# ishine/dmel_codec

Measured on AMD Instinct MI355X. Metric: audio-sec/sec (encode+decode RTF) @24 kHz batch 32, higher is better.
Workload: dtype f32; 1 GPU; cfg2: encode+decode, 24000 Hz, 80 mel, 8 FSQ groups [7, 5, 5], WaveNet 20+20 layers, BigVGAN-base, batch 32 x 1 s per GPU; lanes=3, vocoder_streams=1

## Files before the change

dmel_codec_amd/_lib.py:

```python
from __future__ import annotations

import ctypes as C
import os
from typing import Optional, Sequence

import torch

_HERE = os.path.dirname(os.path.abspath(__file__))
LIB_PATH = os.environ.get("DMEL_LIB") or os.path.join(_HERE, "libdmel_hip.so")
_lib: Optional[C.CDLL] = None

i64p = C.POINTER(C.c_int64)
i32p = C.POINTER(C.c_int32)
f32p = C.POINTER(C.c_float)
vp = C.c_void_p
GRAD_READY_FN = C.CFUNCTYPE(None, vp, C.c_int64, C.c_int64)


class BigVGANConfig(C.Structure):
    _fields_ = [
        ("num_mels", C.c_int),
        ("upsample_initial_channel", C.c_int),
        ("num_upsamples", C.c_int),
        ("upsample_rates", C.c_int * 8),
# ... 10 lines not shown


PROTOTYPES = {
    "dmel_last_error": (C.c_char_p, []),
    "dmel_abi_version": (C.c_int, []),
    "dmel_stft_plan_create": (C.c_int, [C.POINTER(vp), C.c_int, C.c_int, C.c_int, C.c_int, C.c_int, C.c_double, C.c_double, vp]),
    "dmel_stft_plan_destroy": (None, [vp]),
    "dmel_mel_basis_host": (C.c_int, [C.c_int, C.c_int, C.c_int, C.c_double, C.c_double, vp]),
    "dmel_stft_plan_mel_basis": (C.c_int, [vp, vp]),
    "dmel_stft_num_frames": (C.c_int64, [vp, C.c_int64]),
    "dmel_stft_logmel_f32": (C.c_int, [vp, vp, C.c_int64, vp, vp, C.c_int, C.c_int64, vp]),
    "dmel_resample_f32": (C.c_int, [vp, vp, vp, C.c_int, C.c_int64, C.c_int64, C.c_int, C.c_int, C.c_int, vp]),
    "dmel_resample_window_f32": (C.c_int, [vp, C.c_int64, C.c_int64, C.c_int64, vp, vp, C.c_int, C.c_int64, C.c_int64, C.c_int64, C.c_int, C.c_int,
                                           C.c_int, vp]),
    "dmel_resample_window_items_f32": (C.c_int, [vp, C.c_int64, C.c_int64, i64p, i64p, vp, C.c_int64, i64p, vp, C.c_int64, i64p, C.c_int, i64p,
                                                 C.c_int, i64p, i64p, i64p, vp, vp]),
    "dmel_pcm_convert_items": (C.c_int, [C.POINTER(vp), i32p, C.POINTER(vp), i32p, i64p, C.c_int, vp, vp]),
    "dmel_pcm_convert_items_ch": (C.c_int, [C.POINTER(vp), i32p, i32p, i32p, C.POINTER(vp), i32p, i32p, i64p, C.c_int, vp, vp]),
    "dmel_stft_f32": (C.c_int, [vp, vp, C.c_int64, vp, vp, vp, C.c_int, C.c_int64, vp]),
    "dmel_stft_window_f32": (C.c_int, [vp, vp, C.c_int64, C.c_int64, C.c_int64, vp, vp, vp, C.c_int, C.c_int64, C.c_int64, C.c_int64, vp]),
    "dmel_stft_window_items_f32": (C.c_int, [vp, vp, C.c_int64, C.c_int64, i64p, i64p, vp, vp, vp, C.c_int, i64p, i64p, i64p, vp, vp]),
    "dmel_aa_snake_f32": (C.c_int, [vp, vp, vp, vp, vp, vp, C.c_int, C.c_int, C.c_int, C.c_int64, vp]),
    "dmel_aa_snake_items_f32": (C.c_int, [vp, vp, vp, vp, vp, vp, C.c_int, C.c_int, C.c_int, C.c_int64, vp, vp]),
    "dmel_aa_snake_backward_f32": (C.c_int, [vp, vp, vp, vp, vp, vp, vp, vp, vp, C.c_int, C.c_int, C.c_int, C.c_int64, vp]),
    "dmel_discriminator_create": (C.c_int, [C.POINTER(vp)]),
    "dmel_discriminator_destroy": (None, [vp]),
    "dmel_discriminator_set_tensor": (C.c_int, [vp, C.c_char_p, vp, C.POINTER(C.c_int64), C.c_int]),
    "dmel_discriminator_finalize": (C.c_int, [vp]),
    "dmel_discriminator_out_frames": (C.c_int64, [vp, C.c_int64]),
    "dmel_discriminator_workspace_bytes": (C.c_size_t, [vp, C.c_int, C.c_int, C.c_int64]),
    "dmel_discriminator_forward": (C.c_int, [vp, vp, vp, C.c_int, C.c_int, C.c_int64, vp, C.c_size_t, vp]),
    "dmel_discriminator_enable_training": (C.c_int, [vp, C.c_int]),
    "dmel_discriminator_set_train_precision": (C.c_int, [vp, C.c_int]),
    "dmel_discriminator_refresh": (C.c_int, [vp, C.c_int, C.POINTER(C.c_char_p), C.POINTER(vp), vp]),
    "dmel_discriminator_train_workspace_bytes": (C.c_size_t, [vp, C.c_int, C.c_int, C.c_int64]),
    "dmel_discriminator_grad_floats": (C.c_int64, [vp]),
    "dmel_discriminator_grad_slot": (C.c_int, [vp, C.c_char_p, C.POINTER(C.c_int64), C.POINTER(C.c_int64)]),
    "dmel_discriminator_forward_train": (C.c_int, [vp, vp, vp, C.c_int, C.c_int, C.c_int64, vp, C.c_size_t, vp]),
    "dmel_discriminator_backward": (C.c_int, [vp, vp, vp, vp, C.c_int, C.c_int, C.c_int64, vp, C.c_size_t, vp]),
    "dmel_convnext_create": (C.c_int, [C.POINTER(vp), C.c_int]),
    "dmel_convnext_destroy": (None, [vp]),
    "dmel_convnext_set_tensor": (C.c_int, [vp, C.c_char_p, vp, C.POINTER(C.c_int64), C.c_int]),
    "dmel_convnext_enable_training": (C.c_int, [vp, C.c_int]),
    "dmel_convnext_set_train_precision": (C.c_int, [vp, C.c_int]),
    "dmel_convnext_finalize": (C.c_int, [vp]),
    "dmel_convnext_workspace_bytes": (C.c_size_t, [vp, C.c_int, C.c_int64]),
# ... 171 lines not shown
```

dmel_codec_amd/csrc/aa_snake.hip:

```cpp
#include "ops.h"
#include "snake_dev.h"

namespace dmel {

constexpr int kSnakeTile = 1024;
constexpr int kSnakeFwdTile = 1008;

typedef float f32x4 __attribute__((ext_vector_type(4)));

template <bool VEC>
__device__ __forceinline__ void aa_snake_row(const float* __restrict__ xr, float* __restrict__ yr, const float* __restrict__ alpha,
                                             const float* __restrict__ beta, const Taps12& tu, const Taps12& td, int logscale, int c, int T,
                                             int first, int nsub, float* xs, float* ve, float* vo) {
  float a = alpha[c], bt = beta ? beta[c] : a;
  if (logscale) {
    bt = beta ? expf(bt) : expf(a);
    a = expf(a);
  }
  const float inv_b = 1.0f / (bt + 1e-9f);
  const int tid = threadIdx.x;
  auto fetch = [&](int t0) {
    const int s = t0 - 8 + 4 * tid;
    if (VEC && s >= 0 && s + 4 <= T) return *reinterpret_cast<const f32x4*>(xr + s);
    f32x4 v;
    v.x = xr[min(max(s, 0), T - 1)];
    v.y = xr[min(max(s + 1, 0), T - 1)];
    v.z = xr[min(max(s + 2, 0), T - 1)];
    v.w = xr[min(max(s + 3, 0), T - 1)];
    return v;
  };
  float aa[8], bb[8];
#pragma unroll
  for (int i = 0; i < 8; ++i) { aa[i] = a; bb[i] = inv_b; }
  f32x4 pre = {0.f, 0.f, 0.f, 0.f};
  if (first < T) pre = fetch(first);
  for (int sub = 0; sub < nsub; ++sub) {
    const int t0 = first + sub * kSnakeFwdTile;
    if (t0 >= T) break;
    const int len = min(kSnakeFwdTile, T - t0);
    if (sub) __syncthreads();
    *reinterpret_cast<f32x4*>(xs + 4 * tid) = pre;
    if (sub + 1 < nsub && t0 + kSnakeFwdTile < T) pre = fetch(t0 + kSnakeFwdTile);
    __syncthreads();
    if (4 * tid < len + 6) {
      float w[12];
      lds_read3_b128(xs + 4 * tid, w);
      float u[8];
#pragma unroll
      for (int i = 0; i < 4; ++i) {
        float ue = 0.f, uo = 0.f;
#pragma unroll
        for (int j = 0; j < 6; ++j) {
          ue = fmaf(tu.f[2 * j + 1], w[i + 7 - j], ue);
          uo = fmaf(tu.f[2 * j], w[i + 8 - j], uo);
        }
        u[2 * i] = ue;
        u[2 * i + 1] = uo;
      }
      snake_n(u, aa, bb);
      *reinterpret_cast<f32x4*>(ve + 4 * tid) = f32x4{u[0], u[2], u[4], u[6]};
      *reinterpret_cast<f32x4*>(vo + 4 * tid) = f32x4{u[1], u[3], u[5], u[7]};
    }
    __syncthreads();
    const int pe = T - t0 + 3;
    if (t0 == 0 || pe < len + 6) {
      if (tid < 3) {
        if (t0 == 0) ve[tid] = vo[tid] = ve[3];
        if (pe + tid < len + 6) ve[pe + tid] = vo[pe + tid] = vo[pe - 1];
      }
      __syncthreads();
    }
    if (4 * tid < len) {
      float e[12], o[12];
      lds_read3_b128(ve + 4 * tid, e);
      lds_read3_b128(vo + 4 * tid, o);
      f32x4 out;
#pragma unroll
      for (int i = 0; i < 4; ++i) {
        float acc = td.f[0] * o[i];
#pragma unroll
        for (int k = 1; k < 6; ++k) {
          acc = fmaf(td.f[2 * k - 1], e[i + k], acc);
          acc = fmaf(td.f[2 * k], o[i + k], acc);
        }
        out[i] = fmaf(td.f[11], e[i + 6], acc);
      }
      float* yp = yr + t0 + 4 * tid;
      if (VEC) {
        *reinterpret_cast<f32x4*>(yp) = out;
      } else {
#pragma unroll
        for (int i = 0; i < 4; ++i)
          if (4 * tid + i < len) yp[i] = out[i];
      }
    }
  }
}

template <bool VEC>
__global__ __launch_bounds__(256) void aa_snake_kernel(const float* __restrict__ x, float* __restrict__ y,
                                                          const float* __restrict__ alpha, const float* __restrict__ beta,
                                                          Taps12 tu, Taps12 td, int logscale, int C, int T, int nsub) {
  __shared__ __attribute__((aligned(16))) float xs[kSnakeFwdTile + 16];
  __shared__ __attribute__((aligned(16))) float ve[kSnakeFwdTile + 16];
  __shared__ __attribute__((aligned(16))) float vo[kSnakeFwdTile + 16];
  const int c = blockIdx.y, b = blockIdx.z;
  const int64_t row = ((int64_t)b * C + c) * T;
  aa_snake_row<VEC>(x + row, y + row, alpha, beta, tu, td, logscale, c, T, blockIdx.x * nsub * kSnakeFwdTile, nsub, xs, ve, vo);
}

__global__ __launch_bounds__(256) void aa_snake_items_kernel(const float* __restrict__ x, float* __restrict__ y,
                                                                const float* __restrict__ alpha, const float* __restrict__ beta,
                                                                Taps12 tu, Taps12 td, int logscale, int C, int T,
                                                                const int64_t* __restrict__ len, int nsub) {
  __shared__ __attribute__((aligned(16))) float xs[kSnakeFwdTile + 16];
  __shared__ __attribute__((aligned(16))) float ve[kSnakeFwdTile + 16];
  __shared__ __attribute__((aligned(16))) float vo[kSnakeFwdTile + 16];
  const int c = blockIdx.y, b = blockIdx.z;
  const int n = (int)min(max(len[b], (int64_t)0), (int64_t)T);
  const int first = blockIdx.x * nsub * kSnakeFwdTile;
  if (first >= n) return;
  const int64_t row = ((int64_t)b * C + c) * T;
  const float* xr = x + row;
  float* yr = y + row;
  const bool vec = n % 4 == 0 && (reinterpret_cast<uintptr_t>(xr) | reinterpret_cast<uintptr_t>(yr)) % 16 == 0;
  if (vec) aa_snake_row<true>(xr, yr, alpha, beta, tu, td, logscale, c, n, first, nsub, xs, ve, vo);
  else aa_snake_row<false>(xr, yr, alpha, beta, tu, td, logscale, c, n, first, nsub, xs, ve, vo);
}

template <bool PARAMS>
__global__ __launch_bounds__(256) void aa_snake_bwd_kernel(const float* __restrict__ x, const float* __restrict__ dy,
                                                            float* dx, const float* __restrict__ alpha,
                                                            const float* __restrict__ beta, float* __restrict__ dalpha,
                                                            float* __restrict__ dbeta, const float* __restrict__ radd, const float* racc,
                                                            Taps12 tu, Taps12 td, int logscale, int C, int T) {
  __shared__ float xs[kSnakeTile + 12];
  __shared__ float dys[kSnakeTile + 12];
  __shared__ float dvs[2 * (kSnakeTile + 6)];
  __shared__ float dxs[kSnakeTile];
  __shared__ float red[2][4];
  const int c = blockIdx.y, b = blockIdx.z, tid = threadIdx.x;
  const int t0 = blockIdx.x * kSnakeTile;
  const int len = min(kSnakeTile, T - t0);
  const float* xr = x + ((int64_t)b * C + c) * T;
  const float* dyr = dy + ((int64_t)b * C + c) * T;
  float* dxr = dx + ((int64_t)b * C + c) * T;
  float a = alpha[c], bt = beta ? beta[c] : a;
  if (logscale) {
    bt = beta ? expf(bt) : expf(a);
    a = expf(a);
// ... 131 lines not shown
                       (const float*)nullptr, tu, td, logscale, C, (int)T);
  }
  DMEL_HIP(hipGetLastError());
  return DMEL_OK;
}

int launch_aa_snake_bwd_input(const float* x, const float* dy, float* dx, const float* radd, const float* racc, const float* alpha,
                              const float* beta, const float* up_taps_host, const float* down_taps_host, int logscale, int B, int C,
                              int64_t T, hipStream_t s) {
  DMEL_CHECK_ARG(x && dy && dx && alpha && up_taps_host && down_taps_host, "aa_snake_backward_input: NULL argument");
  DMEL_CHECK_ARG(B > 0 && C > 0 && T > 0 && B <= 65535 && C <= 65535 && T < ((int64_t)1 << 29), "aa_snake_backward_input: bad shape");
  Taps12 tu, td;
  for (int i = 0; i < 12; ++i) { tu.f[i] = 2.f * up_taps_host[i]; td.f[i] = down_taps_host[i]; }
  dim3 grid((unsigned)((T + kSnakeTile - 1) / kSnakeTile), (unsigned)C, (unsigned)B);
  {
    ProfScope ps("aa_snake_bwd", s, 0.0, (12.0 + (radd ? 4.0 : 0.0) + (racc ? 4.0 : 0.0)) * (double)B * C * (double)T);
    hipLaunchKernelGGL(aa_snake_bwd_kernel<false>, grid, dim3(256), 0, s, x, dy, dx, alpha, beta, (float*)nullptr, (float*)nullptr, radd,
                       racc, tu, td, logscale, C, (int)T);
  }
  DMEL_HIP(hipGetLastError());
  return DMEL_OK;
}

int launch_aa_snake(const float* x, float* y, const float* alpha, const float* beta, const float* up_taps_host,
                    const float* down_taps_host, int logscale, int B, int C, int64_t T, hipStream_t s) {
  DMEL_CHECK_ARG(x && y && alpha && up_taps_host && down_taps_host, "aa_snake: NULL argument");
  DMEL_CHECK_ARG(B > 0 && C > 0 && T > 0 && B <= 65535 && C <= 65535 && T < ((int64_t)1 << 30), "aa_snake: bad shape");
  Taps12 tu, td;
  for (int i = 0; i < 12; ++i) { tu.f[i] = 2.f * up_taps_host[i]; td.f[i] = down_taps_host[i]; }
  constexpr int nsub = 3;
  constexpr int span = kSnakeFwdTile * nsub;
  dim3 grid((unsigned)((T + span - 1) / span), (unsigned)C, (unsigned)B);
  const bool vec = T % 4 == 0 && (reinterpret_cast<uintptr_t>(x) | reinterpret_cast<uintptr_t>(y)) % 16 == 0;
  {
    ProfScope ps("aa_snake", s, 0.0, 8.0 * (double)B * C * (double)T);
    if (vec) hipLaunchKernelGGL(aa_snake_kernel<true>, grid, dim3(256), 0, s, x, y, alpha, beta, tu, td, logscale, C, (int)T, nsub);
    else hipLaunchKernelGGL(aa_snake_kernel<false>, grid, dim3(256), 0, s, x, y, alpha, beta, tu, td, logscale, C, (int)T, nsub);
  }
  DMEL_HIP(hipGetLastError());
  return DMEL_OK;
}

int launch_aa_snake_items(const float* x, float* y, const float* alpha, const float* beta, const float* up_taps_host,
                          const float* down_taps_host, int logscale, int B, int C, int64_t T, const int64_t* len, hipStream_t s) {
  DMEL_CHECK_ARG(x && y && alpha && up_taps_host && down_taps_host && len, "aa_snake_items: NULL argument");
  DMEL_CHECK_ARG(B > 0 && C > 0 && T > 0 && B <= 65535 && C <= 65535 && T < ((int64_t)1 << 30), "aa_snake_items: bad shape");
  Taps12 tu, td;
  for (int i = 0; i < 12; ++i) { tu.f[i] = 2.f * up_taps_host[i]; td.f[i] = down_taps_host[i]; }
  constexpr int nsub = 3;
  constexpr int span = kSnakeFwdTile * nsub;
  dim3 grid((unsigned)((T + span - 1) / span), (unsigned)C, (unsigned)B);
  {
    ProfScope ps("aa_snake", s, 0.0, 8.0 * (double)B * C * (double)T);
    hipLaunchKernelGGL(aa_snake_items_kernel, grid, dim3(256), 0, s, x, y, alpha, beta, tu, td, logscale, C, (int)T, len, nsub);
  }
  DMEL_HIP(hipGetLastError());
  return DMEL_OK;
}

}

extern "C" int dmel_aa_snake_items_f32(const float* x, float* y, const float* alpha, const float* beta, const float* up_filter12_host,
                                       const float* down_filter12_host, int logscale, int B, int C, int64_t T, const int64_t* lengths_dev,
                                       void* stream) {
  return dmel::launch_aa_snake_items(x, y, alpha, beta, up_filter12_host, down_filter12_host, logscale, B, C, T, lengths_dev,
                                     (hipStream_t)stream);
}

extern "C" int dmel_aa_snake_backward_f32(const float* x, const float* dy, float* dx, const float* alpha, const float* beta,
                                          float* dalpha, float* dbeta, const float* up_filter12_host, const float* down_filter12_host,
                                          int logscale, int B, int C, int64_t T, void* stream) {
  return dmel::launch_aa_snake_bwd(x, dy, dx, alpha, beta, dalpha, dbeta, up_filter12_host, down_filter12_host, logscale, B, C, T,
                                   (hipStream_t)stream);
}

extern "C" int dmel_aa_snake_backward_input_f32(const float* x, const float* dy, const float* add , float* dx, const float* alpha,
                                                const float* beta, const float* up_filter12_host, const float* down_filter12_host,
                                                int logscale, int B, int C, int64_t T, void* stream) {
  return dmel::launch_aa_snake_bwd_input(x, dy, dx, add, nullptr, alpha, beta, up_filter12_host, down_filter12_host, logscale, B, C, T,
                                         (hipStream_t)stream);
}

extern "C" int dmel_aa_snake_f32(const float* x, float* y, const float* alpha, const float* beta, const float* up_filter12_host,
                                 const float* down_filter12_host, int logscale, int B, int C, int64_t T, void* stream) {
  return dmel::launch_aa_snake(x, y, alpha, beta, up_filter12_host, down_filter12_host, logscale, B, C, T, (hipStream_t)stream);
}
```

dmel_codec_amd/csrc/modules.hip:

```cpp
#include <cmath>
#include <cstdlib>
#include <map>
#include <memory>

#include "ops.h"

using namespace dmel;

namespace {

struct HostTensor {
  std::vector<float> v;
  std::vector<int64_t> shape;
  int64_t numel() const { return (int64_t)v.size(); }
};

struct TensorStore {
  std::map<std::string, HostTensor> t;
  int set(const char* key, const float* data, const int64_t* shape, int ndim) {
    DMEL_CHECK_ARG(key && data && shape && ndim >= 0 && ndim <= 4, "set_tensor: bad argument");
    HostTensor h;
    int64_t n = 1;
    for (int i = 0; i < ndim; ++i) { h.shape.push_back(shape[i]); n *= shape[i]; }
    h.v.assign(data, data + n);
// ... 2511 lines not shown
  float* ua = bufs[4];

  {
    ConvRun r = run_1seg(mel, c.num_mels, T, x, c.upsample_initial_channel, T, B);
    r.seg[0].in_len = len_at(0);
    r.precision = prec;
    DMEL_TRY(launch_conv(m->conv_pre, r, st));
  }
  int64_t Tc = T;
  int ch = c.upsample_initial_channel;
  for (int i = 0; i < c.num_upsamples; ++i) {
    const UpStage& us = m->ups[i];
    const int64_t Tn = Tc * us.u;
    DMEL_TRY(launch_up_stage(us, x, xu, B, Tc, prec, st, len_at(i)));
    ch = us.Cout;
    Tc = Tn;
    const int64_t bs = (int64_t)ch * Tc;
    const bool multi = m->multi;
    const int64_t* len = len_at(i + 1);
    if (multi) {
      DMEL_HIP(hipEventRecord(m->ev_fork, st));
      for (int k = 0; k < dmel_bigvgan::kSide; ++k) DMEL_HIP(hipStreamWaitEvent(m->side[k], m->ev_fork, 0));
    }
    for (int j = 0; j < c.num_kernels; ++j) {
      const AmpBlock& ab = m->blocks[(size_t)i * c.num_kernels + j];
      hipStream_t sj = (multi && j > 0) ? m->side[j - 1] : st;
      float *xj = bufs[3 + 3 * j], *uj = bufs[4 + 3 * j], *vj = bufs[5 + 3 * j];
      const float* xin = xu;
      const char* fuse_env = getenv("DMEL_FUSE_SNAKE");
      const bool fuse = fuse_env && fuse_env[0] == '1' && !lengths;
      for (int l = 0; l < 3; ++l) {
        if (l == 0 && multi && j > 0) DMEL_HIP(hipStreamWaitEvent(sj, m->ev_stag[j - 1], 0));
        if (c.resblock_type == 2) {
          ConvRun r2 = run_1seg(uj, ch, Tc, l < 2 ? xj : xs, ch, Tc, B);
          r2.seg[0].in_len = len;
          r2.res = xin; r2.res_bs = bs; r2.res_cs = Tc;
          r2.precision = prec;
          const bool fuse2 = fuse && conv_snake_eligible(ab.c1[l], r2);
          if (!fuse2) DMEL_TRY(act(xin, uj, ab.act[l], ch, Tc, len, sj));
          if (!fuse2 && l == 0 && multi && j + 1 < c.num_kernels) DMEL_HIP(hipEventRecord(m->ev_stag[j], sj));
          if (l == 2) {
            r2.accumulate = j > 0;
            if (j == c.num_kernels - 1) r2.out_div = (float)c.num_kernels;
            if (multi && j > 0) DMEL_HIP(hipStreamWaitEvent(sj, m->ev_chain[j - 1], 0));
          }
          if (fuse2) {
            r2.seg[0].x = xin;
            DMEL_TRY(launch_conv_snake(ab.c1[l], r2, ab.act[l].alpha.as<float>(), ab.act[l].beta.as<float>(), m->taps_up, m->taps_dn, logscale, sj));
            if (l == 0 && multi && j + 1 < c.num_kernels) DMEL_HIP(hipEventRecord(m->ev_stag[j], sj));
          } else {
            DMEL_TRY(launch_conv(ab.c1[l], r2, sj));
          }
          if (l == 2 && multi && j + 1 < c.num_kernels) DMEL_HIP(hipEventRecord(m->ev_chain[j], sj));
          xin = xj;
          continue;
        }
        ConvRun r1 = run_1seg(uj, ch, Tc, vj, ch, Tc, B);
        r1.seg[0].in_len = len;
        r1.precision = prec;
        if (fuse && conv_snake_eligible(ab.c1[l], r1)) {
          r1.seg[0].x = xin;
          DMEL_TRY(launch_conv_snake(ab.c1[l], r1, ab.act[2 * l].alpha.as<float>(), ab.act[2 * l].beta.as<float>(), m->taps_up, m->taps_dn, logscale, sj));
          if (l == 0 && multi && j + 1 < c.num_kernels) DMEL_HIP(hipEventRecord(m->ev_stag[j], sj));
        } else {
          DMEL_TRY(act(xin, uj, ab.act[2 * l], ch, Tc, len, sj));
          if (l == 0 && multi && j + 1 < c.num_kernels) DMEL_HIP(hipEventRecord(m->ev_stag[j], sj));
          DMEL_TRY(launch_conv(ab.c1[l], r1, sj));
        }
        ConvRun r2 = run_1seg(uj, ch, Tc, l < 2 ? xj : xs, ch, Tc, B);
        r2.seg[0].in_len = len;
        r2.res = xin; r2.res_bs = bs; r2.res_cs = Tc;
        r2.precision = prec;
        const bool fuse2 = fuse && conv_snake_eligible(ab.c2[l], r2);
        if (!fuse2) DMEL_TRY(act(vj, uj, ab.act[2 * l + 1], ch, Tc, len, sj));
        if (l == 2) {
          r2.accumulate = j > 0;
          if (j == c.num_kernels - 1) r2.out_div = (float)c.num_kernels;
          if (multi && j > 0) DMEL_HIP(hipStreamWaitEvent(sj, m->ev_chain[j - 1], 0));
        }
        if (fuse2) {
          r2.seg[0].x = vj;
          DMEL_TRY(launch_conv_snake(ab.c2[l], r2, ab.act[2 * l + 1].alpha.as<float>(), ab.act[2 * l + 1].beta.as<float>(), m->taps_up, m->taps_dn, logscale, sj));
        } else {
          DMEL_TRY(launch_conv(ab.c2[l], r2, sj));
        }
        if (l == 2 && multi && j + 1 < c.num_kernels) DMEL_HIP(hipEventRecord(m->ev_chain[j], sj));
        xin = xj;
      }
    }
    if (multi) {
      for (int k = 0; k < dmel_bigvgan::kSide && k + 1 < c.num_kernels; ++k) {
        DMEL_HIP(hipEventRecord(m->ev_join[k], m->side[k]));
        DMEL_HIP(hipStreamWaitEvent(st, m->ev_join[k], 0));
      }
    }
    std::swap(x, xs);
  }
  const int64_t* len_out = len_at(c.num_upsamples);
  DMEL_TRY(act(x, ua, m->act_post, ch, Tc, len_out, st));
  return launch_conv_post(ua, audio, m->post_w.as<float>(), m->post_bias, c.use_tanh_at_final ? ACT_TANH : ACT_CLAMP1, B, ch, 7,
                          Tc, st, len_out);
}

extern "C" int dmel_bigvgan_forward(const dmel_bigvgan* m, const float* mel, float* audio, int B, int64_t T, void* workspace,
                                    size_t workspace_bytes, void* stream) {
  return bigvgan_forward_impl(m, mel, nullptr, audio, B, T, workspace, workspace_bytes, stream);
}

extern "C" int dmel_bigvgan_forward_items(const dmel_bigvgan* m, const float* mel, const int64_t* lengths_dev, float* audio, int B, int64_t T,
                                          void* workspace, size_t workspace_bytes, void* stream) {
  DMEL_CHECK_ARG(lengths_dev, "bigvgan_forward_items: NULL lengths");
  return bigvgan_forward_impl(m, mel, lengths_dev, audio, B, T, workspace, workspace_bytes, stream);
}

extern "C" int dmel_bigvgan_enable_input_grad(dmel_bigvgan* m, int on) {
  DMEL_CHECK_ARG(m, "bigvgan_enable_input_grad: NULL handle");
  if (!m->ready) { set_error("bigvgan_enable_input_grad: handle not finalized"); return DMEL_EMISSING; }
  const dmel_bigvgan_config& c = m->cfg;
  if (!on) {
    m->input_grad = false;
    m->conv_preT = PackedConv();
// ... 243 lines not shown
```

dmel_codec_amd/csrc/ops.h:

```cpp
#pragma once
#include "conv.h"

namespace dmel {

struct FsqConst {
  int n_levels;
  int levels[4], half_width[4], basis[4];
  float half_l[4], offset[4], shift[4];
  int prebound;
  int strict;
};

int make_fsq_const(FsqConst& k, const int* levels, int n, int prebound);
int launch_fsq_encode(const float* z, const float* w_in, const float* b_in, int32_t* ids, float* prequant,
                      const FsqConst& k, int B, int G, int C, int64_t T4, hipStream_t s, const int64_t* len = nullptr);
int launch_fsq_decode(const int32_t* ids, const float* w_out, const float* b_out, float* z, const FsqConst& k, int B,
                      int G, int C, int64_t T4, hipStream_t s, const int64_t* len = nullptr);
int launch_fsq_backward(const float* x, const float* dout, const float* w_in, const float* b_in, const float* w_out, float* dx,
                        float* dw_in, float* db_in, float* dw_out, float* db_out, float* scratch, const FsqConst& k, int B, int G, int C,
                        int64_t T4, hipStream_t s);
int launch_dwconv_ln(const float* x, float* y, const float* dw_w, const float* dw_b, const float* ln_w, const float* ln_b,
                     int N, int C, int64_t T, hipStream_t s, float* h0 = nullptr, const int64_t* len = nullptr, int len_div = 1);
int launch_conv_post(const float* x, float* y, const float* w_dev, float bias, int act, int B, int C, int K, int64_t T,
                     hipStream_t s, const int64_t* len = nullptr);
// ... 18 lines not shown
};
int launch_wavenet_fused(const WaveNetFused& f, const float* x, float* y, const int64_t* in_len, const int64_t* out_len, int len_div, int N,
                         int64_t T, hipStream_t st);
constexpr int kStreamMaxL = 32;
int launch_wavenet_stream(const WaveNetFused& f, const float* x, float* hist, float* skip, float* y, const int64_t* out_len, int len_div,
                          int N, int64_t cap, const int64_t* prev, const int64_t* next, hipStream_t st);
constexpr int kStreamRowInts(int L) { return 2 * (L + 1) + 1; }
int launch_wavenet_stream_items(const WaveNetFused& f, const float* x, float* hist, float* skip, float* y, const int64_t* out_len, int len_div,
                                int N, int64_t cap, const int64_t* prev, const int64_t* next, int32_t* tab_dev, hipStream_t st);
int launch_shift_lengths(const int64_t* len, int64_t shift, int64_t* out, int n, hipStream_t st);
int launch_copy_windows(const float* src, float* dst, int N, int C, int64_t cap, const int32_t* tab, int stride, int i_shift, int i_end,
                        int len_div, int64_t max_cols, int64_t cols_total, hipStream_t st);
int launch_shift_lengths_items(const int64_t* len, const int32_t* tab, int stride, int i_shift, int64_t* out, int n, hipStream_t st);
struct LenScales {
  static constexpr int kMax = 9;
  int64_t v[kMax];
};
int launch_length_tables(const int64_t* len, int64_t* tab, int n, int64_t T, int stages, const LenScales& scale, hipStream_t st);
int launch_stage_lengths(const int64_t* len, int64_t* tab, int n, int64_t T, int stages, int down, hipStream_t st);
int launch_aa_snake(const float* x, float* y, const float* alpha, const float* beta, const float* up_taps_host,
                    const float* down_taps_host, int logscale, int B, int C, int64_t T, hipStream_t s);
int launch_aa_snake_items(const float* x, float* y, const float* alpha, const float* beta, const float* up_taps_host,
                          const float* down_taps_host, int logscale, int B, int C, int64_t T, const int64_t* len, hipStream_t s);
int launch_aa_snake_bwd_input(const float* x, const float* dy, float* dx, const float* radd, const float* racc, const float* alpha,
                              const float* beta, const float* up_taps_host, const float* down_taps_host, int logscale, int B, int C,
                              int64_t T, hipStream_t s);

bool conv_snake_eligible(const PackedConv& pc, const ConvRun& r);
int launch_conv_snake(const PackedConv& pc, const ConvRun& r, const float* alpha, const float* beta, const float* up_taps_host,
                      const float* down_taps_host, int logscale, hipStream_t stream);

bool conv_pc_eligible(const PackedConv& pc, const ConvRun& r, bool any_size = false);
int launch_conv_pc(const PackedConv& pc, const ConvRun& r, hipStream_t stream);

int launch_gate_fwd(const float* pre, float* z, int N, int C, int64_t T, hipStream_t s);
int launch_gate_bwd(const float* dz, const float* pre, float* dpre, int N, int C, int64_t T, hipStream_t s);
int launch_resskip_fwd(const float* x, const float* o, float* xn, float* skipsum, int first, int N, int C, int64_t T, hipStream_t s);
int launch_resskip_bwd(const float* gx, const float* gs, float* go, float* gxs, int N, int C, int64_t T, hipStream_t s);
int launch_silu_fwd(const float* u, float* y, int64_t total, hipStream_t s);
int launch_silu_bwd(const float* g, const float* u, float* du, int64_t total, hipStream_t s);
int launch_scale(const float* x, float* y, float k, int64_t total, hipStream_t s);
int launch_gelu_fwd(const float* u, float* g, int64_t total, hipStream_t s);
int launch_gelu_bwd(const float* dg, const float* u, float* du, int64_t total, hipStream_t s);
int launch_layerscale_res_fwd(const float* x, const float* v, const float* gamma, float* y, int N, int C, int64_t T, hipStream_t s);
int launch_layerscale_bwd(const float* dy, const float* v, const float* gamma, float* dv, float* dgamma, int N, int C, int64_t T,
                          hipStream_t s);
// ... 13 lines not shown
```

include/dmel_hip.h:

```cpp
#ifndef DMEL_HIP_H
#define DMEL_HIP_H

#include <stddef.h>
#include <stdint.h>

#ifdef __cplusplus
extern "C" {
#endif

#define DMEL_OK 0
#define DMEL_EINVAL (-1)
#define DMEL_EUNSUPPORTED (-2)
#define DMEL_EMISSING (-3)

#define DMEL_PRECISION_FP32 0
#define DMEL_PRECISION_BF16 1
#define DMEL_PRECISION_FP32_MFMA 2
#define DMEL_PRECISION_FP32_F16X2 3
#define DMEL_PRECISION_FP32_BF16X3 4

const char* dmel_last_error(void);
int dmel_abi_version(void);

typedef struct dmel_stft_plan dmel_stft_plan;
// ... 35 lines not shown
                                   int64_t bank_arena_floats, const int64_t* rates, int n_rates, const int64_t* rate_index, int B,
                                   const int64_t* o0, const int64_t* n_out, const int64_t* total_length, int64_t* table_scratch,
                                   void* stream);

#define DMEL_SAMPLE_F32 0
#define DMEL_SAMPLE_S16 1
#define DMEL_SAMPLE_ULAW 8
#define DMEL_SAMPLE_ALAW 9
int dmel_pcm_convert_items(const void* const* src, const int32_t* src_fmt, void* const* dst, const int32_t* dst_fmt, const int64_t* n,
                           int B, void* table_scratch, void* stream);
#define DMEL_MAX_CHANNELS 8
int dmel_pcm_convert_items_ch(const void* const* src, const int32_t* src_fmt, const int32_t* src_ch, const int32_t* src_pick,
                              void* const* dst, const int32_t* dst_fmt, const int32_t* dst_ch, const int64_t* n, int B,
                              void* table_scratch, void* stream);

int dmel_collate_peak_f32(const float* const* clips_dev, const int64_t* lengths_dev, const int32_t* order_dev , float* audios,
                          int32_t* audio_lengths, uint32_t* peaks_scratch, int B, int64_t Lmax, float peak, void* stream);

int dmel_aa_snake_f32(const float* x, float* y, const float* alpha, const float* beta, const float* up_filter12_host,
                      const float* down_filter12_host, int logscale, int B, int C, int64_t T, void* stream);
int dmel_aa_snake_items_f32(const float* x, float* y, const float* alpha, const float* beta, const float* up_filter12_host,
                            const float* down_filter12_host, int logscale, int B, int C, int64_t T, const int64_t* lengths_dev,
                            void* stream);
int dmel_aa_snake_backward_f32(const float* x, const float* dy, float* dx, const float* alpha, const float* beta ,
                               float* dalpha, float* dbeta , const float* up_filter12_host,
                               const float* down_filter12_host, int logscale, int B, int C, int64_t T, void* stream);

int dmel_aa_snake_backward_input_f32(const float* x, const float* dy, const float* add , float* dx, const float* alpha,
                                     const float* beta , const float* up_filter12_host, const float* down_filter12_host,
                                     int logscale, int B, int C, int64_t T, void* stream);


typedef struct dmel_wavenet dmel_wavenet;
int dmel_wavenet_create(dmel_wavenet** m, int input_channels , int output_channels ,
                        int residual_channels, int residual_layers, int dilation_cycle, int condition_channels );
void dmel_wavenet_destroy(dmel_wavenet* m);
int dmel_wavenet_set_precision(dmel_wavenet* m, int precision);
int dmel_wavenet_set_tensor(dmel_wavenet* m, const char* key, const float* data_host, const int64_t* shape, int ndim);
int dmel_wavenet_finalize(dmel_wavenet* m);
size_t dmel_wavenet_workspace_bytes(const dmel_wavenet* m, int N, int64_t T);
int dmel_wavenet_forward(const dmel_wavenet* m, const float* x, const float* condition, float* y, int N, int64_t T,
                         const int64_t* in_lengths, const int64_t* out_lengths, int group_repeat,
                         void* workspace, size_t workspace_bytes, void* stream);

int dmel_wavenet_enable_training(dmel_wavenet* m, int on);
int dmel_wavenet_set_train_precision(dmel_wavenet* m, int precision);
// ... 210 lines not shown
```

Measured before the change: 2696 audio-sec/sec.

## Share anti-aliased snake upsample across resblock kernels and fuse post snake with conv

BigVGAN's multi-receptive-field blocks all apply their first anti-aliased snake to the same input. A new multi-set kernel reads and upsamples that input once, then applies each kernel's alpha/beta and downsamples into separate outputs, replacing two or three separate launches. A second new kernel fuses the final snake activation with the 7-tap, C-to-1 post conv and tanh/clamp, so the full-resolution activated tensor is never written to global memory. Both paths are on by default (shared only when not multi-stream). The trade-offs are extra barriers per set, more LDS per block and a serial loop over channels in the post kernel, which may limit parallelism.

```diff
diff --git a/dmel_codec_amd/_lib.py b/dmel_codec_amd/_lib.py
--- a/dmel_codec_amd/_lib.py
+++ b/dmel_codec_amd/_lib.py
@@ -56,6 +56,8 @@
     "dmel_stft_window_items_f32": (C.c_int, [vp, vp, C.c_int64, C.c_int64, i64p, i64p, vp, vp, vp, C.c_int, i64p, i64p, i64p, vp, vp]),
     "dmel_aa_snake_f32": (C.c_int, [vp, vp, vp, vp, vp, vp, C.c_int, C.c_int, C.c_int, C.c_int64, vp]),
     "dmel_aa_snake_items_f32": (C.c_int, [vp, vp, vp, vp, vp, vp, C.c_int, C.c_int, C.c_int, C.c_int64, vp, vp]),
+    "dmel_aa_snake_shared_f32": (C.c_int, [vp, C.c_int, vp, vp, vp, vp, vp, C.c_int, C.c_int, C.c_int, C.c_int64, vp, vp]),
+    "dmel_snake_post_f32": (C.c_int, [vp, vp, vp, vp, C.c_float, C.c_int, vp, vp, vp, C.c_int, C.c_int, C.c_int, C.c_int64, vp, vp]),
     "dmel_aa_snake_backward_f32": (C.c_int, [vp, vp, vp, vp, vp, vp, vp, vp, vp, C.c_int, C.c_int, C.c_int, C.c_int64, vp]),
     "dmel_discriminator_create": (C.c_int, [C.POINTER(vp)]),
     "dmel_discriminator_destroy": (None, [vp]),
diff --git a/dmel_codec_amd/csrc/aa_snake.hip b/dmel_codec_amd/csrc/aa_snake.hip
--- a/dmel_codec_amd/csrc/aa_snake.hip
+++ b/dmel_codec_amd/csrc/aa_snake.hip
@@ -8,16 +8,61 @@
 
 typedef float f32x4 __attribute__((ext_vector_type(4)));
 
-template <bool VEC>
-__device__ __forceinline__ void aa_snake_row(const float* __restrict__ xr, float* __restrict__ yr, const float* __restrict__ alpha,
-                                             const float* __restrict__ beta, const Taps12& tu, const Taps12& td, int logscale, int c, int T,
+__device__ __forceinline__ void aa_up4(const float* xq, const Taps12& tu, float (&u)[8]) {
+  float w[12];
+  lds_read3_b128(xq, w);
+#pragma unroll
+  for (int i = 0; i < 4; ++i) {
+    float ue = 0.f, uo = 0.f;
+#pragma unroll
+    for (int j = 0; j < 6; ++j) {
+      ue = fmaf(tu.f[2 * j + 1], w[i + 7 - j], ue);
+      uo = fmaf(tu.f[2 * j], w[i + 8 - j], uo);
+    }
+    u[2 * i] = ue;
+    u[2 * i + 1] = uo;
+  }
+}
+__device__ __forceinline__ f32x4 aa_down4(const float* eq, const float* oq, const Taps12& td) {
+  float e[12], o[12];
+  lds_read3_b128(eq, e);
+  lds_read3_b128(oq, o);
+  f32x4 out;
+#pragma unroll
+  for (int i = 0; i < 4; ++i) {
+    float acc = td.f[0] * o[i];
+#pragma unroll
+    for (int k = 1; k < 6; ++k) {
+      acc = fmaf(td.f[2 * k - 1], e[i + k], acc);
+      acc = fmaf(td.f[2 * k], o[i + k], acc);
+    }
+    out[i] = fmaf(td.f[11], e[i + 6], acc);
+  }
+  return out;
+}
+
+template <int NS> struct SnakeSets {
+  const float* alpha[NS];
+  const float* beta[NS];
+  float* y[NS];
+};
+
+template <bool VEC, int NS>
+__device__ __forceinline__ void aa_snake_row(const float* __restrict__ xr, float* __restrict__ const (&yr)[NS], const SnakeSets<NS>& ps,
+                                             const Taps12& tu, const Taps12& td, int logscale, int c, int T,
                                              int first, int nsub, float* xs, float* ve, float* vo) {
-  float a = alpha[c], bt = beta ? beta[c] : a;
-  if (logscale) {
-    bt = beta ? expf(bt) : expf(a);
-    a = expf(a);
-  }
-  const float inv_b = 1.0f / (bt + 1e-9f);
+  float a[NS], inv_b[NS];
+#pragma unroll
+  for (int i = 0; i < NS; ++i) {
+    const float* beta = ps.beta[i];
+    float bt = beta ? beta[c] : ps.alpha[i][c];
+    a[i] = ps.alpha[i][c];
+    if (logscale) {
+      bt = beta ? expf(bt) : expf(a[i]);
+      a[i] = expf(a[i]);
+    }
+    inv_b[i] = 1.0f / (bt + 1e-9f);
+  }
   const int tid = threadIdx.x;
   auto fetch = [&](int t0) {
     const int s = t0 - 8 + 4 * tid;
@@ -29,9 +74,6 @@
     v.w = xr[min(max(s + 3, 0), T - 1)];
     return v;
   };
-  float aa[8], bb[8];
-#pragma unroll
-  for (int i = 0; i < 8; ++i) { aa[i] = a; bb[i] = inv_b; }
   f32x4 pre = {0.f, 0.f, 0.f, 0.f};
   if (first < T) pre = fetch(first);
   for (int sub = 0; sub < nsub; ++sub) {
@@ -42,77 +84,62 @@
     *reinterpret_cast<f32x4*>(xs + 4 * tid) = pre;
     if (sub + 1 < nsub && t0 + kSnakeFwdTile < T) pre = fetch(t0 + kSnakeFwdTile);
     __syncthreads();
-    if (4 * tid < len + 6) {
-      float w[12];
-      lds_read3_b128(xs + 4 * tid, w);
-      float u[8];
-#pragma unroll
-      for (int i = 0; i < 4; ++i) {
-        float ue = 0.f, uo = 0.f;
-#pragma unroll
-        for (int j = 0; j < 6; ++j) {
-          ue = fmaf(tu.f[2 * j + 1], w[i + 7 - j], ue);
-          uo = fmaf(tu.f[2 * j], w[i + 8 - j], uo);
+    float u[8];
+#pragma unroll
+    for (int set = 0; set < NS; ++set) {
+      if (set) __syncthreads();
+      if (4 * tid < len + 6) {
+        if (set == 0) {
+          aa_up4(xs + 4 * tid, tu, u);
         }
-        u[2 * i] = ue;
-        u[2 * i + 1] = uo;
-      }
-      snake_n(u, aa, bb);
-      *reinterpret_cast<f32x4*>(ve + 4 * tid) = f32x4{u[0], u[2], u[4], u[6]};
-      *reinterpret_cast<f32x4*>(vo + 4 * tid) = f32x4{u[1], u[3], u[5], u[7]};
-    }
-    __syncthreads();
-    const int pe = T - t0 + 3;
-    if (t0 == 0 || pe < len + 6) {
-      if (tid < 3) {
-        if (t0 == 0) ve[tid] = vo[tid] = ve[3];
-        if (pe + tid < len + 6) ve[pe + tid] = vo[pe + tid] = vo[pe - 1];
+        float v[8], aa[8], bb[8];
+#pragma unroll
+        for (int i = 0; i < 8; ++i) { v[i] = u[i]; aa[i] = a[set]; bb[i] = inv_b[set]; }
+        snake_n(v, aa, bb);
+        *reinterpret_cast<f32x4*>(ve + 4 * tid) = f32x4{v[0], v[2], v[4], v[6]};
+        *reinterpret_cast<f32x4*>(vo + 4 * tid) = f32x4{v[1], v[3], v[5], v[7]};
       }
       __syncthreads();
-    }
-    if (4 * tid < len) {
-      float e[12], o[12];
-      lds_read3_b128(ve + 4 * tid, e);
-      lds_read3_b128(vo + 4 * tid, o);
-      f32x4 out;
-#pragma unroll
-      for (int i = 0; i < 4; ++i) {
-        float acc = td.f[0] * o[i];
-#pragma unroll
-        for (int k = 1; k < 6; ++k) {
-          acc = fmaf(td.f[2 * k - 1], e[i + k], acc);
-          acc = fmaf(td.f[2 * k], o[i + k], acc);
+      const int pe = T - t0 + 3;
+      if (t0 == 0 || pe < len + 6) {
+        if (tid < 3) {
+          if (t0 == 0) ve[tid] = vo[tid] = ve[3];
+          if (pe + tid < len + 6) ve[pe + tid] = vo[pe + tid] = vo[pe - 1];
         }
-        out[i] = fmaf(td.f[11], e[i + 6], acc);
-      }
-      float* yp = yr + t0 + 4 * tid;
-      if (VEC) {
-        *reinterpret_cast<f32x4*>(yp) = out;
-      } else {
-#pragma unroll
-        for (int i = 0; i < 4; ++i)
-          if (4 * tid + i < len) yp[i] = out[i];
-      }
-    }
-  }
-}
-
-template <bool VEC>
-__global__ __launch_bounds__(256) void aa_snake_kernel(const float* __restrict__ x, float* __restrict__ y,
-                                                          const float* __restrict__ alpha, const float* __restrict__ beta,
-                                                          Taps12 tu, Taps12 td, int logscale, int C, int T, int nsub) {
+        __syncthreads();
+      }
+      if (4 * tid < len) {
+        const f32x4 out = aa_down4(ve + 4 * tid, vo + 4 * tid, td);
+        float* yp = yr[set] + t0 + 4 * tid;
+        if (VEC) {
+          *reinterpret_cast<f32x4*>(yp) = out;
+        } else {
+#pragma unroll
+          for (int i = 0; i < 4; ++i)
+            if (4 * tid + i < len) yp[i] = out[i];
+        }
+      }
+    }
+  }
+}
+
+template <bool VEC, int NS>
+__global__ __launch_bounds__(256) void aa_snake_kernel(const float* __restrict__ x, SnakeSets<NS> ps, Taps12 tu, Taps12 td, int logscale,
+                                                          int C, int T, int nsub) {
   __shared__ __attribute__((aligned(16))) float xs[kSnakeFwdTile + 16];
   __shared__ __attribute__((aligned(16))) float ve[kSnakeFwdTile + 16];
   __shared__ __attribute__((aligned(16))) float vo[kSnakeFwdTile + 16];
   const int c = blockIdx.y, b = blockIdx.z;
   const int64_t row = ((int64_t)b * C + c) * T;
-  aa_snake_row<VEC>(x + row, y + row, alpha, beta, tu, td, logscale, c, T, blockIdx.x * nsub * kSnakeFwdTile, nsub, xs, ve, vo);
-}
-
-__global__ __launch_bounds__(256) void aa_snake_items_kernel(const float* __restrict__ x, float* __restrict__ y,
-                                                                const float* __restrict__ alpha, const float* __restrict__ beta,
-                                                                Taps12 tu, Taps12 td, int logscale, int C, int T,
-                                                                const int64_t* __restrict__ len, int nsub) {
+  float* yr[NS];
+#pragma unroll
+  for (int i = 0; i < NS; ++i) yr[i] = ps.y[i] + row;
+  aa_snake_row<VEC, NS>(x + row, yr, ps, tu, td, logscale, c, T, blockIdx.x * nsub * kSnakeFwdTile, nsub, xs, ve, vo);
+}
+
+template <int NS>
+__global__ __launch_bounds__(256) void aa_snake_items_kernel(const float* __restrict__ x, SnakeSets<NS> ps, Taps12 tu, Taps12 td,
+                                                                int logscale, int C, int T, const int64_t* __restrict__ len, int nsub) {
   __shared__ __attribute__((aligned(16))) float xs[kSnakeFwdTile + 16];
   __shared__ __attribute__((aligned(16))) float ve[kSnakeFwdTile + 16];
   __shared__ __attribute__((aligned(16))) float vo[kSnakeFwdTile + 16];
@@ -122,10 +149,116 @@
   if (first >= n) return;
   const int64_t row = ((int64_t)b * C + c) * T;
   const float* xr = x + row;
-  float* yr = y + row;
-  const bool vec = n % 4 == 0 && (reinterpret_cast<uintptr_t>(xr) | reinterpret_cast<uintptr_t>(yr)) % 16 == 0;
-  if (vec) aa_snake_row<true>(xr, yr, alpha, beta, tu, td, logscale, c, n, first, nsub, xs, ve, vo);
-  else aa_snake_row<false>(xr, yr, alpha, beta, tu, td, logscale, c, n, first, nsub, xs, ve, vo);
+  float* yr[NS];
+  uintptr_t bits = reinterpret_cast<uintptr_t>(xr);
+#pragma unroll
+  for (int i = 0; i < NS; ++i) {
+    yr[i] = ps.y[i] + row;
+    bits |= reinterpret_cast<uintptr_t>(yr[i]);
+  }
+  const bool vec = n % 4 == 0 && bits % 16 == 0;
+  if (vec) aa_snake_row<true, NS>(xr, yr, ps, tu, td, logscale, c, n, first, nsub, xs, ve, vo);
+  else aa_snake_row<false, NS>(xr, yr, ps, tu, td, logscale, c, n, first, nsub, xs, ve, vo);
+}
+
+constexpr int kPostFusedTile = 1000;
+template <bool VEC>
+__global__ __launch_bounds__(256) void snake_post_kernel(const float* __restrict__ x, float* __restrict__ y, const float* __restrict__ alpha,
+                                                          const float* __restrict__ beta, const float* __restrict__ w, float bias,
+                                                          Taps12 tu, Taps12 td, int logscale, int C, int T, int act,
+                                                          const int64_t* __restrict__ len) {
+  __shared__ __attribute__((aligned(16))) float xs[kSnakeFwdTile + 16];
+  __shared__ __attribute__((aligned(16))) float ve[kSnakeFwdTile + 16];
+  __shared__ __attribute__((aligned(16))) float vo[kSnakeFwdTile + 16];
+  __shared__ __attribute__((aligned(16))) float ys[kSnakeFwdTile + 16];
+  extern __shared__ float wsm[];
+  const int b = blockIdx.y, tid = threadIdx.x;
+  const int t0 = blockIdx.x * kPostFusedTile;
+  const int n = len ? (int)min(max(len[b], (int64_t)0), (int64_t)T) : T;
+  float* yb = y + (int64_t)b * T;
+  if (t0 >= n) {
+    for (int t = t0 + tid; t < min(t0 + kPostFusedTile, T); t += 256) yb[t] = 0.f;
+    return;
+  }
+  for (int i = tid; i < C * 7; i += 256) wsm[i] = w[i];
+  const int ta = t0 - 4;
+  const int alen = min(kSnakeFwdTile, n - ta);
+  const float* xb = x + (int64_t)b * C * T;
+  auto fetch = [&](const float* xr) {
+    const int s = ta - 8 + 4 * tid;
+    if (VEC && s >= 0 && s + 4 <= n) return *reinterpret_cast<const f32x4*>(xr + s);
+    f32x4 v;
+    v.x = xr[min(max(s, 0), n - 1)];
+    v.y = xr[min(max(s + 1, 0), n - 1)];
+    v.z = xr[min(max(s + 2, 0), n - 1)];
+    v.w = xr[min(max(s + 3, 0), n - 1)];
+    return v;
+  };
+  float acc[4] = {bias, bias, bias, bias};
+  f32x4 pre = fetch(xb);
+  for (int c = 0; c < C; ++c) {
+    float a = alpha[c], bt = beta ? beta[c] : a;
+    if (logscale) {
+      bt = beta ? expf(bt) : expf(a);
+      a = expf(a);
+    }
+    const float inv_b = 1.0f / (bt + 1e-9f);
+    *reinterpret_cast<f32x4*>(xs + 4 * tid) = pre;
+    if (c + 1 < C) pre = fetch(xb + (int64_t)(c + 1) * T);
+    __syncthreads();
+    if (4 * tid < alen + 6) {
+      float u[8], aa[8], bb[8];
+      aa_up4(xs + 4 * tid, tu, u);
+#pragma unroll
+      for (int i = 0; i < 8; ++i) { aa[i] = a; bb[i] = inv_b; }
+      snake_n(u, aa, bb);
+      *reinterpret_cast<f32x4*>(ve + 4 * tid) = f32x4{u[0], u[2], u[4], u[6]};
+      *reinterpret_cast<f32x4*>(vo + 4 * tid) = f32x4{u[1], u[3], u[5], u[7]};
+    }
+    __syncthreads();
+    const int p0 = 3 - ta;
+    const int pe = n - ta + 3;
+    if (ta < 0 || pe < alen + 6) {
+      if (tid < 3) {
+        if (ta < 0) ve[p0 - 3 + tid] = vo[p0 - 3 + tid] = ve[p0];
+        if (pe + tid < alen + 6) ve[pe + tid] = vo[pe + tid] = vo[pe - 1];
+      }
+      __syncthreads();
+    }
+    if (tid < kSnakeFwdTile / 4) {
+      f32x4 out = {0.f, 0.f, 0.f, 0.f};
+      if (4 * tid < alen) {
+        out = aa_down4(ve + 4 * tid, vo + 4 * tid, td);
+#pragma unroll
+        for (int i = 0; i < 4; ++i) {
+          const int col = ta + 4 * tid + i;
+          if (col < 0 || col >= n) out[i] = 0.f;
+        }
+      }
+      *reinterpret_cast<f32x4*>(ys + 4 * tid) = out;
+    }
+    __syncthreads();
+    if (tid < kPostFusedTile / 4) {
+      float v[12];
+      lds_read3_b128(ys + 4 * tid, v);
+#pragma unroll
+      for (int k = 0; k < 7; ++k) {
+        const float wv = wsm[c * 7 + k];
+#pragma unroll
+        for (int e = 0; e < 4; ++e) acc[e] = fmaf(wv, v[e + 1 + k], acc[e]);
+      }
+    }
+  }
+  if (tid < kPostFusedTile / 4) {
+#pragma unroll
+    for (int e = 0; e < 4; ++e) {
+      const int t = t0 + 4 * tid + e;
+      if (t < T) {
+        const float v = act == 2 ? tanhf(acc[e]) : (act == 3 ? fminf(fmaxf(acc[e], -1.f), 1.f) : acc[e]);
+        yb[t] = t < n ? v : 0.f;
+      }
+    }
+  }
 }
 
 template <bool PARAMS>
@@ -303,37 +436,69 @@
   return DMEL_OK;
 }
 
-int launch_aa_snake(const float* x, float* y, const float* alpha, const float* beta, const float* up_taps_host,
-                    const float* down_taps_host, int logscale, int B, int C, int64_t T, hipStream_t s) {
-  DMEL_CHECK_ARG(x && y && alpha && up_taps_host && down_taps_host, "aa_snake: NULL argument");
+template <int NS>
+static int launch_aa_snake_sets(const float* x, float* const* y, const float* const* alpha, const float* const* beta, const Taps12& tu,
+                                const Taps12& td, int logscale, int B, int C, int64_t T, const int64_t* len, hipStream_t s) {
+  SnakeSets<NS> ps;
+  uintptr_t bits = reinterpret_cast<uintptr_t>(x);
+  for (int i = 0; i < NS; ++i) {
+    ps.alpha[i] = alpha[i]; ps.beta[i] = beta[i]; ps.y[i] = y[i];
+    bits |= reinterpret_cast<uintptr_t>(y[i]);
+  }
+  constexpr int nsub = 3;
+  constexpr int span = kSnakeFwdTile * nsub;
+  dim3 grid((unsigned)((T + span - 1) / span), (unsigned)C, (unsigned)B);
+  const bool vec = T % 4 == 0 && bits % 16 == 0;
+  {
+    ProfScope ps_("aa_snake", s, 0.0, 4.0 * (1 + NS) * (double)B * C * (double)T);
+    if (len) hipLaunchKernelGGL(aa_snake_items_kernel<NS>, grid, dim3(256), 0, s, x, ps, tu, td, logscale, C, (int)T, len, nsub);
+    else if (vec) hipLaunchKernelGGL((aa_snake_kernel<true, NS>), grid, dim3(256), 0, s, x, ps, tu, td, logscale, C, (int)T, nsub);
+    else hipLaunchKernelGGL((aa_snake_kernel<false, NS>), grid, dim3(256), 0, s, x, ps, tu, td, logscale, C, (int)T, nsub);
+  }
+  DMEL_HIP(hipGetLastError());
+  return DMEL_OK;
+}
+
+int launch_aa_snake_shared(const float* x, int nsets, float* const* y, const float* const* alpha, const float* const* beta,
+                           const float* up_taps_host, const float* down_taps_host, int logscale, int B, int C, int64_t T,
+                           const int64_t* len, hipStream_t s) {
+  DMEL_CHECK_ARG(x && y && alpha && beta && up_taps_host && down_taps_host, "aa_snake: NULL argument");
+  DMEL_CHECK_ARG(nsets >= 1 && nsets <= 3, "aa_snake: 1 to 3 parameter sets");
+  for (int i = 0; i < nsets; ++i) DMEL_CHECK_ARG(y[i] && alpha[i], "aa_snake: NULL argument");
   DMEL_CHECK_ARG(B > 0 && C > 0 && T > 0 && B <= 65535 && C <= 65535 && T < ((int64_t)1 << 30), "aa_snake: bad shape");
   Taps12 tu, td;
   for (int i = 0; i < 12; ++i) { tu.f[i] = 2.f * up_taps_host[i]; td.f[i] = down_taps_host[i]; }
-  constexpr int nsub = 3;
-  constexpr int span = kSnakeFwdTile * nsub;
-  dim3 grid((unsigned)((T + span - 1) / span), (unsigned)C, (unsigned)B);
-  const bool vec = T % 4 == 0 && (reinterpret_cast<uintptr_t>(x) | reinterpret_cast<uintptr_t>(y)) % 16 == 0;
-  {
-    ProfScope ps("aa_snake", s, 0.0, 8.0 * (double)B * C * (double)T);
-    if (vec) hipLaunchKernelGGL(aa_snake_kernel<true>, grid, dim3(256), 0, s, x, y, alpha, beta, tu, td, logscale, C, (int)T, nsub);
-    else hipLaunchKernelGGL(aa_snake_kernel<false>, grid, dim3(256), 0, s, x, y, alpha, beta, tu, td, logscale, C, (int)T, nsub);
-  }
-  DMEL_HIP(hipGetLastError());
-  return DMEL_OK;
+  if (nsets == 1) return launch_aa_snake_sets<1>(x, y, alpha, beta, tu, td, logscale, B, C, T, len, s);
+  if (nsets == 2) return launch_aa_snake_sets<2>(x, y, alpha, beta, tu, td, logscale, B, C, T, len, s);
+  return launch_aa_snake_sets<3>(x, y, alpha, beta, tu, td, logscale, B, C, T, len, s);
+}
+
+int launch_aa_snake(const float* x, float* y, const float* alpha, const float* beta, const float* up_taps_host,
+                    const float* down_taps_host, int logscale, int B, int C, int64_t T, hipStream_t s) {
+  return launch_aa_snake_shared(x, 1, &y, &alpha, &beta, up_taps_host, down_taps_host, logscale, B, C, T, nullptr, s);
 }
 
 int launch_aa_snake_items(const float* x, float* y, const float* alpha, const float* beta, const float* up_taps_host,
                           const float* down_taps_host, int logscale, int B, int C, int64_t T, const int64_t* len, hipStream_t s) {
-  DMEL_CHECK_ARG(x && y && alpha && up_taps_host && down_taps_host && len, "aa_snake_items: NULL argument");
-  DMEL_CHECK_ARG(B > 0 && C > 0 && T > 0 && B <= 65535 && C <= 65535 && T < ((int64_t)1 << 30), "aa_snake_items: bad shape");
+  DMEL_CHECK_ARG(len, "aa_snake_items: NULL argument");
+  return launch_aa_snake_shared(x, 1, &y, &alpha, &beta, up_taps_host, down_taps_host, logscale, B, C, T, len, s);
+}
+
+int launch_snake_post(const float* x, float* y, const float* alpha, const float* beta, const float* w_dev, float bias, int act,
+                      const float* up_taps_host, const float* down_taps_host, int logscale, int B, int C, int64_t T, const int64_t* len,
+                      hipStream_t s) {
+  DMEL_CHECK_ARG(x && y && alpha && w_dev && up_taps_host && down_taps_host, "snake_post: NULL argument");
+  DMEL_CHECK_ARG(B > 0 && B <= 65535 && C > 0 && T > 0 && T < ((int64_t)1 << 30), "snake_post: bad shape");
+  const size_t lds = (size_t)C * 7 * sizeof(float);
+  DMEL_CHECK_ARG(lds <= 32 * 1024, "snake_post: weight table too large");
   Taps12 tu, td;
   for (int i = 0; i < 12; ++i) { tu.f[i] = 2.f * up_taps_host[i]; td.f[i] = down_taps_host[i]; }
-  constexpr int nsub = 3;
-  constexpr int span = kSnakeFwdTile * nsub;
-  dim3 grid((unsigned)((T + span - 1) / span), (unsigned)C, (unsigned)B);
+  dim3 grid((unsigned)((T + kPostFusedTile - 1) / kPostFusedTile), (unsigned)B);
+  const bool vec = T % 4 == 0 && reinterpret_cast<uintptr_t>(x) % 16 == 0;
   {
-    ProfScope ps("aa_snake", s, 0.0, 8.0 * (double)B * C * (double)T);
-    hipLaunchKernelGGL(aa_snake_items_kernel, grid, dim3(256), 0, s, x, y, alpha, beta, tu, td, logscale, C, (int)T, len, nsub);
+    ProfScope ps("small", s, 0.0, 4.0 * B * (double)T * (C + 1));
+    if (vec) hipLaunchKernelGGL(snake_post_kernel<true>, grid, dim3(256), lds, s, x, y, alpha, beta, w_dev, bias, tu, td, logscale, C, (int)T, act, len);
+    else hipLaunchKernelGGL(snake_post_kernel<false>, grid, dim3(256), lds, s, x, y, alpha, beta, w_dev, bias, tu, td, logscale, C, (int)T, act, len);
   }
   DMEL_HIP(hipGetLastError());
   return DMEL_OK;
@@ -348,6 +513,21 @@
                                      (hipStream_t)stream);
 }
 
+extern "C" int dmel_snake_post_f32(const float* x, const float* alpha, const float* beta, const float* w_dev, float bias, int act, float* y,
+                                   const float* up_filter12_host, const float* down_filter12_host, int logscale, int B, int C, int64_t T,
+                                   const int64_t* lengths_dev, void* stream) {
+  DMEL_CHECK_ARG(act == 0 || act == 2 || act == 3, "snake_post: act must be 0 (none), 2 (tanh) or 3 (clamp to [-1, 1])");
+  return dmel::launch_snake_post(x, y, alpha, beta, w_dev, bias, act, up_filter12_host, down_filter12_host, logscale, B, C, T, lengths_dev,
+                                 (hipStream_t)stream);
+}
+
+extern "C" int dmel_aa_snake_shared_f32(const float* x, int nsets, float* const* y, const float* const* alpha, const float* const* beta,
+                                        const float* up_filter12_host, const float* down_filter12_host, int logscale, int B, int C, int64_t T,
+                                        const int64_t* lengths_dev, void* stream) {
+  return dmel::launch_aa_snake_shared(x, nsets, y, alpha, beta, up_filter12_host, down_filter12_host, logscale, B, C, T, lengths_dev,
+                                      (hipStream_t)stream);
+}
+
 extern "C" int dmel_aa_snake_backward_f32(const float* x, const float* dy, float* dx, const float* alpha, const float* beta,
                                           float* dalpha, float* dbeta, const float* up_filter12_host, const float* down_filter12_host,
                                           int logscale, int B, int C, int64_t T, void* stream) {
diff --git a/dmel_codec_amd/csrc/modules.hip b/dmel_codec_amd/csrc/modules.hip
--- a/dmel_codec_amd/csrc/modules.hip
+++ b/dmel_codec_amd/csrc/modules.hip
@@ -2557,13 +2557,24 @@
       DMEL_HIP(hipEventRecord(m->ev_fork, st));
       for (int k = 0; k < dmel_bigvgan::kSide; ++k) DMEL_HIP(hipStreamWaitEvent(m->side[k], m->ev_fork, 0));
     }
+    const char* fuse_env = getenv("DMEL_FUSE_SNAKE");
+    const bool fuse = fuse_env && fuse_env[0] == '1' && !lengths;
+    const char* shared_env = getenv("DMEL_SNAKE_SHARED");
+    const bool shared = !(shared_env && shared_env[0] == '0') && !multi && !fuse && c.num_kernels >= 2 && c.num_kernels <= 3;
+    if (shared) {
+      float* ys[3];
+      const float *al[3], *be[3];
+      for (int j = 0; j < c.num_kernels; ++j) {
+        const SnakeP& p = m->blocks[(size_t)i * c.num_kernels + j].act[0];
+        ys[j] = bufs[4 + 3 * j]; al[j] = p.alpha.as<float>(); be[j] = p.beta.as<float>();
+      }
+      DMEL_TRY(launch_aa_snake_shared(xu, c.num_kernels, ys, al, be, m->taps_up, m->taps_dn, logscale, B, ch, Tc, len, st));
+    }
     for (int j = 0; j < c.num_kernels; ++j) {
       const AmpBlock& ab = m->blocks[(size_t)i * c.num_kernels + j];
       hipStream_t sj = (multi && j > 0) ? m->side[j - 1] : st;
       float *xj = bufs[3 + 3 * j], *uj = bufs[4 + 3 * j], *vj = bufs[5 + 3 * j];
       const float* xin = xu;
-      const char* fuse_env = getenv("DMEL_FUSE_SNAKE");
-      const bool fuse = fuse_env && fuse_env[0] == '1' && !lengths;
       for (int l = 0; l < 3; ++l) {
         if (l == 0 && multi && j > 0) DMEL_HIP(hipStreamWaitEvent(sj, m->ev_stag[j - 1], 0));
         if (c.resblock_type == 2) {
@@ -2572,7 +2583,7 @@
           r2.res = xin; r2.res_bs = bs; r2.res_cs = Tc;
           r2.precision = prec;
           const bool fuse2 = fuse && conv_snake_eligible(ab.c1[l], r2);
-          if (!fuse2) DMEL_TRY(act(xin, uj, ab.act[l], ch, Tc, len, sj));
+          if (!fuse2 && !(shared && l == 0)) DMEL_TRY(act(xin, uj, ab.act[l], ch, Tc, len, sj));
           if (!fuse2 && l == 0 && multi && j + 1 < c.num_kernels) DMEL_HIP(hipEventRecord(m->ev_stag[j], sj));
           if (l == 2) {
             r2.accumulate = j > 0;
@@ -2598,7 +2609,7 @@
           DMEL_TRY(launch_conv_snake(ab.c1[l], r1, ab.act[2 * l].alpha.as<float>(), ab.act[2 * l].beta.as<float>(), m->taps_up, m->taps_dn, logscale, sj));
           if (l == 0 && multi && j + 1 < c.num_kernels) DMEL_HIP(hipEventRecord(m->ev_stag[j], sj));
         } else {
-          DMEL_TRY(act(xin, uj, ab.act[2 * l], ch, Tc, len, sj));
+          if (!(shared && l == 0)) DMEL_TRY(act(xin, uj, ab.act[2 * l], ch, Tc, len, sj));
           if (l == 0 && multi && j + 1 < c.num_kernels) DMEL_HIP(hipEventRecord(m->ev_stag[j], sj));
           DMEL_TRY(launch_conv(ab.c1[l], r1, sj));
         }
@@ -2632,6 +2643,10 @@
     std::swap(x, xs);
   }
   const int64_t* len_out = len_at(c.num_upsamples);
+  const char* post_env = getenv("DMEL_POST_FUSED");
+  if (!(post_env && post_env[0] == '0'))
+    return launch_snake_post(x, audio, m->act_post.alpha.as<float>(), m->act_post.beta.as<float>(), m->post_w.as<float>(), m->post_bias,
+                             c.use_tanh_at_final ? ACT_TANH : ACT_CLAMP1, m->taps_up, m->taps_dn, logscale, B, ch, Tc, len_out, st);
   DMEL_TRY(act(x, ua, m->act_post, ch, Tc, len_out, st));
   return launch_conv_post(ua, audio, m->post_w.as<float>(), m->post_bias, c.use_tanh_at_final ? ACT_TANH : ACT_CLAMP1, B, ch, 7,
                           Tc, st, len_out);
diff --git a/dmel_codec_amd/csrc/ops.h b/dmel_codec_amd/csrc/ops.h
--- a/dmel_codec_amd/csrc/ops.h
+++ b/dmel_codec_amd/csrc/ops.h
@@ -64,6 +64,12 @@
                     const float* down_taps_host, int logscale, int B, int C, int64_t T, hipStream_t s);
 int launch_aa_snake_items(const float* x, float* y, const float* alpha, const float* beta, const float* up_taps_host,
                           const float* down_taps_host, int logscale, int B, int C, int64_t T, const int64_t* len, hipStream_t s);
+int launch_aa_snake_shared(const float* x, int nsets, float* const* y, const float* const* alpha, const float* const* beta,
+                           const float* up_taps_host, const float* down_taps_host, int logscale, int B, int C, int64_t T,
+                           const int64_t* len, hipStream_t s);
+int launch_snake_post(const float* x, float* y, const float* alpha, const float* beta, const float* w_dev, float bias, int act,
+                      const float* up_taps_host, const float* down_taps_host, int logscale, int B, int C, int64_t T, const int64_t* len,
+                      hipStream_t s);
 int launch_aa_snake_bwd_input(const float* x, const float* dy, float* dx, const float* radd, const float* racc, const float* alpha,
                               const float* beta, const float* up_taps_host, const float* down_taps_host, int logscale, int B, int C,
                               int64_t T, hipStream_t s);
diff --git a/include/dmel_hip.h b/include/dmel_hip.h
--- a/include/dmel_hip.h
+++ b/include/dmel_hip.h
@@ -81,6 +81,12 @@
 int dmel_aa_snake_items_f32(const float* x, float* y, const float* alpha, const float* beta, const float* up_filter12_host,
                             const float* down_filter12_host, int logscale, int B, int C, int64_t T, const int64_t* lengths_dev,
                             void* stream);
+int dmel_aa_snake_shared_f32(const float* x, int nsets, float* const* y, const float* const* alpha, const float* const* beta,
+                             const float* up_filter12_host, const float* down_filter12_host, int logscale, int B, int C, int64_t T,
+                             const int64_t* lengths_dev, void* stream);
+int dmel_snake_post_f32(const float* x, const float* alpha, const float* beta, const float* w_dev, float bias, int act, float* y,
+                        const float* up_filter12_host, const float* down_filter12_host, int logscale, int B, int C, int64_t T,
+                        const int64_t* lengths_dev, void* stream);
 int dmel_aa_snake_backward_f32(const float* x, const float* dy, float* dx, const float* alpha, const float* beta ,
                                float* dalpha, float* dbeta , const float* up_filter12_host,
                                const float* down_filter12_host, int logscale, int B, int C, int64_t T, void* stream);
```

New measurement: 2709 audio-sec/sec, median of 6. No clear change (+0.5%).
